# NCAR/SPERR

Measured on AMD Instinct MI355X. Metric: compress+decompress GB/s/GPU on 256^3 fp32 chunks @ BPP=2.0; bitstream-exact vs ref, higher is better.
Workload: dtype f64; 1 GPU; synthetic 1024^3 fp32 turbulence per GPU, 256^3 chunks, BPP=2.0, step = compress + decompress, volume and container resident in HBM; chunks_per_gpu=64, parallelism=chunks farmed over 1 GPU(s), no collective

## Files before the change

### sperr_amd/csrc/xform.hip

```cpp
#include <type_traits>

#include "xform.h"
#include "lift_window.h"
#include "dequant.h"

namespace sperrhip {


constexpr int kSumStrides = 64, kSumSeg = 64;


template <typename T>
__global__ void __launch_bounds__(kThreads)
k_stride_sums(const T* __restrict__ vol, VolDesc vd, const ChunkGeom* geom, uint32_t cx,
              uint32_t cy, uint32_t cz, uint32_t nstrides, uint32_t ssz, double* strideMean,
              size_t strideMeanStride, CoderState* st, int want_range)
{
  __shared__ double tile[kSumStrides][kSumSeg + 1];
  __shared__ uint32_t sh_differs;
  double vmax = -INFINITY, vnegmax = -INFINITY;
  const uint32_t c = blockIdx.y;
  const uint32_t s0 = blockIdx.x * kSumStrides;
  const ChunkGeom g = geom[c];
  const size_t vx = vd.dims[0], vy = vd.dims[1];
  const T first = vol[((size_t)g.org[2] * vy + g.org[1]) * vx + g.org[0]];
  if (threadIdx.x == 0)
    sh_differs = 0;
  double acc = 0.0;
  bool differs = false;
  (void)cz;
  for (uint32_t seg = 0; seg < ssz; seg += kSumSeg) {
    const uint32_t len = min((uint32_t)kSumSeg, ssz - seg);
    __syncthreads();
    for (uint32_t k = threadIdx.x; k < (uint32_t)(kSumStrides * kSumSeg); k += kThreads) {
      const uint32_t r = k / kSumSeg, j = k % kSumSeg;
      const uint32_t sidx = s0 + r;
      if (sidx < nstrides && j < len) {
        const uint32_t e = sidx * ssz + seg + j;
        const uint32_t x = e % cx, q = e / cx;
        const uint32_t y = q % cy, z = q / cy;
        const T v = vol[((size_t)(g.org[2] + z) * vy + (g.org[1] + y)) * vx + g.org[0] + x];
        differs |= (v != first);
        tile[r][j] = (double)v;
        vmax = fmax(vmax, (double)v);
        vnegmax = fmax(vnegmax, -(double)v);
      }
    }
    __syncthreads();
    if (threadIdx.x < (uint32_t)kSumStrides && s0 + threadIdx.x < nstrides)
      for (uint32_t j = 0; j < len; j++)
        acc += tile[threadIdx.x][j];
  }
  if (differs)
    sh_differs = 1;
  __syncthreads();
  if (threadIdx.x < (uint32_t)kSumStrides && s0 + threadIdx.x < nstrides)
    strideMean[c * strideMeanStride + s0 + threadIdx.x] = acc / (double)ssz;
  if (threadIdx.x == 0 && sh_differs)
    st[c].not_const_flag = 1;
  if (want_range) {
    for (int d = 32; d > 0; d >>= 1) {
      vmax = fmax(vmax, __shfl_xor(vmax, d, 64));
      vnegmax = fmax(vnegmax, __shfl_xor(vnegmax, d, 64));
    }
    if ((threadIdx.x & 63) == 0) {
      atomicMax(reinterpret_cast<unsigned long long*>(&st[c].vmaxKey), order_key(vmax));
      atomicMax(reinterpret_cast<unsigned long long*>(&st[c].vnegmaxKey), order_key(vnegmax));
    }
  }
}

template <typename T>
__global__ void __launch_bounds__(64)
k_stride_sums_rows(const T* __restrict__ vol, VolDesc vd, const ChunkGeom* geom, uint32_t cx,
                   uint32_t cy, uint32_t nstrides, uint32_t ssz, double* strideMean,
                   size_t strideMeanStride, CoderState* st, int want_range)
{
  constexpr int V = 16 / sizeof(T);
  struct alignas(16) Pack { T v[V]; };
  const uint32_t c = blockIdx.y;
  const uint32_t sidx = blockIdx.x * 64 + threadIdx.x;
  const ChunkGeom g = geom[c];
  const size_t vx = vd.dims[0], vy = vd.dims[1];
  const T first = vol[((size_t)g.org[2] * vy + g.org[1]) * vx + g.org[0]];
  double acc = 0.0, vmax = -INFINITY, vnegmax = -INFINITY;
  bool differs = false;
// ... 288 lines not shown
    }
    else {
      if (l < nl)
        for (uint32_t i = k0; i < odd_len; i += kg)
          OD(i) = (-K.eps) * OD(i);
      __syncthreads();
      if (l < nl)
        for (uint32_t i = k0; i < even_len; i += kg) {
          const uint32_t a = max(i, 1u) - 1, b = min(i, odd_len - 1);
          const double t = K.delta * (OD(a) + OD(b));
          EV(i) = fma(EV(i), K.inv_eps, -t);
        }
      __syncthreads();
      odd_step(-K.gamma);
      even_step(-K.beta);
      odd_step(-K.alpha);
    }
#undef EV
#undef OD
  }

  auto crop_store = [&](uint32_t l, uint32_t p, VT v) {
    uint32_t xyz[3];
    xyz[axis] = p;
    xyz[ua] = u0 + l;
    xyz[wa] = tw;
    if (crop_has(cg, xyz[0], xyz[1], xyz[2]))
      vol[crop_addr(cg, vd, xyz[0], xyz[1], xyz[2])] = v;
  };
  (void)crop_store;
  const bool wantMax = FORWARD && F.mode == 1 && !is_const;
  double vmax = 0.0;
  if (axis == 0) {
    const uint32_t nseg = (len + 63) / 64;
    for (uint32_t sg = tid / 64; sg < nl * nseg; sg += kThreads / 64) {
      const uint32_t l = sg / nseg, p = (sg % nseg) * 64 + tid % 64;
      if (p >= len)
        continue;
      const uint32_t src = FORWARD ? p : ((p & 1) ? even_len + (p >> 1) : (p >> 1));
      if constexpr (kCrop)
        crop_store(l, p, (VT)(is_const ? mean : sm[src * NLP + l] + mean));
      else if (IO != 0 && !FORWARD)
        vol[vbase + l * vsu + p * vsl] = (VT)(is_const ? mean : sm[src * NLP + l] + mean);
      else {
        const double v = sm[src * NLP + l];
        tile[l * su + p] = v;
        size_t idx;
        if (wantMax && outside_inner(l, p, idx))
          vmax = fmax(vmax, fabs(v));
      }
    }
  }
  else {
    const uint32_t l = tid % NL, k0 = tid / NL, kg = kThreads / NL;
    if (l < nl)
      for (uint32_t p = k0; p < len; p += kg) {
        const uint32_t src = FORWARD ? p : ((p & 1) ? even_len + (p >> 1) : (p >> 1));
        if constexpr (kCrop)
          crop_store(l, p, (VT)(is_const ? mean : sm[src * NLP + l] + mean));
        else if (IO != 0 && !FORWARD)
          vol[vbase + l * vsu + p * vsl] = (VT)(is_const ? mean : sm[src * NLP + l] + mean);
        else {
          const double v = sm[src * NLP + l];
          tile[l * su + p * sl] = v;
          size_t idx;
          if (wantMax && outside_inner(l, p, idx))
            vmax = fmax(vmax, fabs(v));
        }
      }
  }
  if (FORWARD && F.mode == 1) {
    for (int d = 32; d > 0; d >>= 1)
      vmax = fmax(vmax, __shfl_xor(vmax, d, 64));
    if ((tid & 63) == 0 && vmax > 0.0)
      atomicMax(reinterpret_cast<unsigned long long*>(&st[c].maxabs),
                (unsigned long long)__double_as_longlong(vmax));
  }
}

constexpr int kXYHalo = 4;
constexpr int kXYThreads = 512;
constexpr int kStage = 16;
constexpr int kSeg = 8;

__device__ __forceinline__ uint32_t reflect_index(int q, int n)
{
  const int period = 2 * (n - 1);
  q = q < 0 ? -q : q;
  if (q >= period)
    q %= period;
  return (uint32_t)(q < n ? q : period - q);
}


template <bool FORWARD, int IO, bool kCrop = false>
__global__ void __launch_bounds__(kXYThreads)
k_lift_xy(double* vals, size_t valsStride, uint32_t cx, uint32_t cy, uint32_t cz, int R,
          LiftConsts K, const CoderState* st, void* volume, VolDesc vd, const GeomOf<kCrop>* geom)
{
  static_assert(IO == 1 || IO == 2, "float or double volume");
  static_assert(!kCrop || !FORWARD, "the crop variant is a last inverse pass");
  using VT = typename std::conditional<IO == 1, float, double>::type;
  const uint32_t c = blockIdx.y;
  const bool is_const = st[c].is_const != 0;
  if (is_const && FORWARD)
    return;
  double* sm = reinterpret_cast<double*>(dyn_smem);
  const uint32_t ntile = (cy + R - 1) / R;
  const uint32_t z = blockIdx.x / ntile, y0 = (blockIdx.x % ntile) * R;
  const uint32_t ylo = y0 >= (uint32_t)kXYHalo ? y0 - kXYHalo : 0u;
  const uint32_t yhi = min(cy, y0 + R + kXYHalo);
  const uint32_t yend = min(cy, y0 + R);
  const uint32_t nrow = yhi - ylo;
  const uint32_t RS = cx + 1;
  const uint32_t xe = cx - cx / 2, ye = cy - cy / 2;
  const GeomOf<kCrop> g = geom[c];
  VT* vol = reinterpret_cast<VT*>(volume);
  const size_t vsy = vd.dims[0], vsz = (size_t)vd.dims[0] * vd.dims[1];
  size_t vbase = 0;
  uint32_t wy0 = y0, wy1 = yend, wx0 = 0, wx1 = cx;
  if constexpr (kCrop) {
    wy0 = max(y0, g.lo[1]);
    wy1 = min(yend, g.hi[1]);
    wx0 = g.lo[0];
    wx1 = g.hi[0];
    if (z - g.lo[2] >= g.hi[2] - g.lo[2] || wy0 >= wy1)
      return;
  }
  else
    vbase = (size_t)(g.org[2] + z) * vsz + (size_t)g.org[1] * vsy + g.org[0];
  auto out_at = [&](uint32_t x, uint32_t y) -> size_t {
    if constexpr (kCrop)
      return crop_addr(g, vd, x, y, z);
    else
      return vbase + (size_t)y * vsy + x;
  };
  double* buf = vals + c * valsStride + (size_t)z * cx * cy;
  const double mean = st[c].mean;
  const uint32_t tid = threadIdx.x;

  if (is_const) {
    if constexpr (kCrop) {
      const uint32_t w = wx1 - wx0;
      for (uint32_t k = tid; k < (wy1 - wy0) * w; k += kXYThreads)
        vol[out_at(wx0 + k % w, wy0 + k / w)] = (VT)mean;
    }
    else
      for (uint32_t k = tid; k < (yend - y0) * cx; k += kXYThreads)
        vol[vbase + (size_t)(y0 + k / cx) * vsy + k % cx] = (VT)mean;
    return;
  }

  const uint32_t lane = tid & 63u, wave = tid >> 6, nwaves = kXYThreads / 64;
  {
    using ST = typename std::conditional<FORWARD, VT, double>::type;
    const uint32_t nxb = (cx + 63) / 64;
    const uint32_t rowsW = nrow > wave ? (nrow - wave + nwaves - 1) / nwaves : 0;
    const uint32_t items = rowsW * nxb;
    uint32_t ri = 0, bi = 0;
    for (uint32_t m0 = 0; m0 < items; m0 += kStage) {
      ST v[kStage];
      uint32_t ri2 = ri, bi2 = bi;
#pragma unroll
      for (int u = 0; u < kStage; u++) {
        const uint32_t j = wave + nwaves * ri2, x = lane + 64 * bi2;
        v[u] = 0;
        if (m0 + u < items && x < cx) {
          const uint32_t y = ylo + j;
          if (FORWARD)
            v[u] = (ST)vol[vbase + (size_t)y * vsy + x];
          else
            v[u] = (ST)buf[(size_t)((y & 1) ? ye + (y >> 1) : (y >> 1)) * cx + ((x & 1) ? xe + (x >> 1) : (x >> 1))];
        }
        if (++bi2 == nxb) {
          bi2 = 0;
// ... 78 lines not shown
        const uint32_t dcol = (x & 1) ? xe + (x >> 1) : (x >> 1);
#pragma unroll
        for (int k = 0; k < kSeg; k++) {
          const uint32_t y = y0 + q * kSeg + k;
          if (y < yend)
            buf[(size_t)((y & 1) ? ye + (y >> 1) : (y >> 1)) * cx + dcol] = r[4 + k];
        }
      }
    }
  }
  else {
    for (uint32_t xb = 0; xb < cx; xb += cpr) {
      const uint32_t x = xb + tid % cpr, q = tid / cpr;
      const bool on = x < cx && q < nq;
      double r[16];
      if (on) {
        load_column(x, q, r);
        lift16<false>(r, K);
      }
      __syncthreads();
      if (on) {
#pragma unroll
        for (int k = 0; k < kSeg; k++) {
          const uint32_t y = y0 + q * kSeg + k;
          if (y < yend)
            sm[(size_t)(y - ylo) * RS + x] = r[4 + k];
        }
      }
    }
    __syncthreads();
    lift_x(y0 - ylo, yend - ylo);
    if constexpr (kCrop) {
      for (uint32_t y = wy0 + wave; y < wy1; y += nwaves) {
        VT* dstrow = vol + out_at(wx0, y);
        const double* srow = sm + (size_t)(y - ylo) * RS;
        for (uint32_t x = wx0 + lane; x < wx1; x += 64)
          dstrow[x - wx0] = (VT)(srow[x] + mean);
      }
    }
    else
    for (uint32_t y = y0 + wave; y < yend; y += nwaves) {
      VT* dstrow = vol + vbase + (size_t)y * vsy;
      const double* srow = sm + (size_t)(y - ylo) * RS;
      for (uint32_t x = lane; x < cx; x += 64)
        dstrow[x] = (VT)(srow[x] + mean);
    }
  }
}

#ifndef XYZ_INV_THREADS
#define XYZ_INV_THREADS 1024
#endif
#ifndef XYZ_INV_PREFETCH
#define XYZ_INV_PREFETCH 2
#endif
#ifndef XYZ_FWD_THREADS
#define XYZ_FWD_THREADS 1024
#endif
constexpr int kXYZThreadsF = XYZ_FWD_THREADS, kXYZThreadsI = XYZ_INV_THREADS;
constexpr int kXYZRows = 16;
constexpr int kXYZStaged = kXYZRows + 2 * kXYHalo;
constexpr int kXYZPosF = (4096 + kXYZThreadsF - 1) / kXYZThreadsF;
constexpr int kXYZStageF = (6144 + kXYZThreadsF - 1) / kXYZThreadsF;
constexpr int kXYZPosI = 6144 / kXYZThreadsI;
#ifndef XYZ_INV_GROUP
#define XYZ_INV_GROUP 3
#endif
constexpr int kXYZGroupI = XYZ_INV_GROUP;
#ifndef XYZ_FWD_YOUT
#define XYZ_FWD_YOUT 4
#endif
#ifndef XYZ_FWD_XOUT
#define XYZ_FWD_XOUT 8
#endif
#ifndef XYZ_INV_YOUT
#define XYZ_INV_YOUT 4
#endif
#ifndef XYZ_INV_XOUT
#define XYZ_INV_XOUT 4
#endif
#ifndef XYZ_INV_XSTORE
#define XYZ_INV_XSTORE 1
#endif
#ifndef XYZ_FWD_OFF
#define XYZ_FWD_OFF 0
#endif
#ifndef XYZ_INV_OFF
#define XYZ_INV_OFF 0
#endif
template <int MASK>
__device__ __forceinline__ bool xyz_off(int bit, uint32_t nseg)
{
  return (MASK & bit) != 0 && nseg != ~0u;
}
constexpr int kXYZOutFY = XYZ_FWD_YOUT, kXYZOutFX = XYZ_FWD_XOUT, kXYZOutIY = XYZ_INV_YOUT, kXYZOutIX = XYZ_INV_XOUT;
constexpr bool xyz_out_ok(int n) { return n == 2 || n == 4 || n == 8; }
static_assert(xyz_out_ok(kXYZOutFY) && xyz_out_ok(kXYZOutFX) && xyz_out_ok(kXYZOutIY) && xyz_out_ok(kXYZOutIX), "2, 4 or 8 outputs a task");
constexpr int kXYZBoxSlots = 48;

__host__ __device__ inline uint32_t xyz_row_stride(uint32_t cx)
{
  return ((cx + 7u) & ~7u) + 9u;
}

#define XYZ_LDS_BARRIER() asm volatile("s_waitcnt lgkmcnt(0)\n\ts_barrier" ::: "memory")

__device__ __forceinline__ void xyz_put(double* row, uint32_t x, uint32_t cx, double v)
{
  row[4 + x] = v;
  if (x - 1u < 4u)
    row[4 - x] = v;
  if (cx - 2u - x < 4u)
    row[2 * cx + 2 - x] = v;
}

template <bool FORWARD, int NT, int NOUT>
__device__ __forceinline__ void xyz_lift_x(const double* src, double* dst, uint32_t RS, uint32_t cx, uint32_t jlo,
                                           uint32_t jhi, uint32_t tid, const LiftConsts& K)
{
  const uint32_t nseg = (cx + NOUT - 1) / NOUT;
  const uint32_t ntask = (jhi - jlo) * nseg;
#pragma unroll 1
  for (uint32_t t = tid; t < ntask; t += NT) {
    const uint32_t rows = jhi - jlo, sg = t / rows, rb = jlo + (t - sg * rows);
    const double* row = src + (size_t)rb * RS + sg * NOUT;
    double r[NOUT + 8];
#pragma unroll
    for (int k = 0; k < NOUT + 8; k++)
      r[k] = row[k];
    lift_window<FORWARD, NOUT + 8>(r, K);
    double* out = dst + (size_t)rb * RS + 4 + sg * NOUT;
#pragma unroll
    for (int k = 0; k < NOUT; k++)
      if (sg * NOUT + k < cx)
        out[k] = r[4 + k];
  }
}

template <int NT, int NOUT, typename VT>
__device__ __forceinline__ void xyz_lift_x_store(const double* src, VT* vrows, size_t vsy, uint32_t RS, uint32_t cx, uint32_t jlo,
                                                 uint32_t jhi, uint32_t tid, const LiftConsts& K, double mean, bool noMean,
                                                 bool doStore)
{
  const uint32_t nseg = (cx + NOUT - 1) / NOUT;
  const uint32_t ntask = (jhi - jlo) * nseg;
#pragma unroll 1
  for (uint32_t t = tid; t < ntask; t += NT) {
    const uint32_t rows = jhi - jlo, sg = t / rows, rb = t - sg * rows;
    const double* row = src + (size_t)(jlo + rb) * RS + sg * NOUT;
    double r[NOUT + 8];
#pragma unroll
    for (int k = 0; k < NOUT + 8; k++)
      r[k] = row[k];
    lift_window<false, NOUT + 8>(r, K);
    VT* out = vrows + (size_t)rb * vsy + sg * NOUT;
    VT v[NOUT];
#pragma unroll
    for (int k = 0; k < NOUT; k++)
      v[k] = (VT)(noMean ? r[4 + k] : r[4 + k] + mean);
    if (!doStore)
      continue;
    if (sg * NOUT + NOUT <= cx) {
      typedef VT Seg __attribute__((ext_vector_type(NOUT), aligned(sizeof(VT))));
      Seg s;
#pragma unroll
      for (int k = 0; k < NOUT; k++)
        s[k] = v[k];
      *reinterpret_cast<Seg*>(out) = s;
    }
    else {
#pragma unroll
      for (int k = 0; k < NOUT; k++)
        if (sg * NOUT + k < cx)
          out[k] = v[k];
    }
  }
}

template <bool FORWARD, bool APRON, int NT, int NOUT>
__device__ __forceinline__ void xyz_lift_y(const double* src, double* dst, uint32_t RS, uint32_t cx, uint32_t nt,
                                           uint32_t tid, const LiftConsts& K)
{
  const uint32_t nq = (nt + NOUT - 1) / NOUT;
  const uint32_t ntask = nq * cx;
#pragma unroll 1
  for (uint32_t t = tid; t < ntask; t += NT) {
    const uint32_t q = t / cx, x = t - q * cx;
    const double* top = src + (size_t)(q * NOUT) * RS + 4 + x;
    double r[NOUT + 8];
#pragma unroll
    for (int k = 0; k < NOUT + 8; k++)
      r[k] = top[(size_t)k * RS];
    lift_window<FORWARD, NOUT + 8>(r, K);
#pragma unroll
    for (int k = 0; k < NOUT; k++) {
      if (q * NOUT + k < nt) {
        double* row = dst + (size_t)(4 + q * NOUT + k) * RS;
        if (APRON)
          xyz_put(row, x, cx, r[4 + k]);
        else
          row[4 + x] = r[4 + k];
      }
    }
  }
}

template <typename VT, int NPOS, int NSTG, bool L2>
__device__ __forceinline__ void xyz_fwd_body(double* buf, const uint32_t orow, const size_t sliceN, uint32_t cx, uint32_t cy,
                                             uint32_t cz, const LiftConsts& K, CoderState* stc, const VT* volc, const size_t vsy,
                                             const size_t vsz, const double mean, int wantMax, uint32_t in0, uint32_t in1,
                                             uint32_t in2, uint32_t nseg, double* box)
{
  const uint32_t tid = threadIdx.x;
  const uint32_t seg = blockIdx.x % nseg, npairsAll = (cz + 1) / 2;
  const uint32_t mA = seg == 0 ? 0u : (uint32_t)((uint64_t)npairsAll * seg / nseg);
  const uint32_t mB = seg + 1 == nseg ? npairsAll : (uint32_t)((uint64_t)npairsAll * (seg + 1) / nseg);
  const uint32_t zFirst = mA >= 6 ? 2 * (mA - 6) : 0u;
  const uint32_t zEnd = seg + 1 == nseg ? cz : 2 * mB - 1;
  const uint32_t y0 = (blockIdx.x / nseg) * kXYZRows;
  const uint32_t nt = min((uint32_t)kXYZRows, cy - y0);
  const uint32_t RS = xyz_row_stride(cx);
  double* sm = reinterpret_cast<double*>(dyn_smem);
  const uint32_t bufN = (uint32_t)kXYZStaged * RS;
  const uint32_t xe = cx - cx / 2, ye = cy - cy / 2, ze = cz - cz / 2;
  const size_t boxSlice = (size_t)in0 * in1;

  const uint32_t nstage = (uint32_t)kXYZStaged * cx;
  uint32_t pk[NSTG];
#pragma unroll
  for (int k = 0; k < NSTG; k++) {
    const uint32_t q = tid + (uint32_t)k * kXYZThreadsF;
    const uint32_t j = q / cx, x = q - j * cx;
    pk[k] = (j << 27) | (reflect_index((int)y0 - kXYHalo + (int)j, (int)cy) << 12) | x;
  }
  const uint32_t npos = nt * cx;
  uint32_t srow[NPOS], ooff[NPOS];
  uint32_t boff[L2 ? 1 : NPOS];
  uint32_t outerMask = 0;
#pragma unroll
  for (int k = 0; k < NPOS; k++) {
    const uint32_t q = tid + (uint32_t)k * kXYZThreadsF;
    const uint32_t row = q / cx, col = q - row * cx, y = y0 + row;
    srow[k] = ((row + kXYHalo) << 16) | col;
    const uint32_t drow = (y & 1) ? ye + (y >> 1) : (y >> 1), dcol = (col & 1) ? xe + (col >> 1) : (col >> 1);
    ooff[k] = drow * orow + dcol;
    if constexpr (!L2)
      boff[k] = drow * in0 + dcol;
    if (!(dcol < in0 && drow < in1))
      outerMask |= 1u << k;
  }
  double sxe[NPOS], sxo[NPOS], d1p[NPOS], e1p[NPOS], d2p[NPOS];
#pragma unroll
  for (int k = 0; k < NPOS; k++)
    sxe[k] = sxo[k] = d1p[k] = e1p[k] = d2p[k] = 0.0;
  double vmax = 0.0;
  auto emit = [&](int k, uint32_t zp, double v) {
    bool toBox = false;
    if constexpr (!L2)
      toBox = box != nullptr && zp < in2 && !((outerMask >> k) & 1u);
    if (!xyz_off<XYZ_FWD_OFF>(4, nseg))
      *(toBox ? box + ((size_t)zp * boxSlice + boff[L2 ? 0 : k]) : buf + ((size_t)zp * sliceN + ooff[k])) = v;
    if (wantMax && (((outerMask >> k) & 1u) || zp >= in2))
      vmax = fmax(vmax, fabs(v));
  };

  VT pre[NSTG];
  auto issue = [&](uint32_t z) {
    const VT* src = volc + (size_t)z * vsz;
#pragma unroll
    for (int k = 0; k < NSTG; k++) {
      if (xyz_off<XYZ_FWD_OFF>(1, nseg)) {
        pre[k] = (VT)(((pk[k] + z * 40503u) * 2654435761u) >> 20);
      }
      else {
        pre[k] = (tid + (uint32_t)k * kXYZThreadsF) < nstage
                     ? src[(size_t)((pk[k] >> 12) & 0x7fffu) * vsy + (pk[k] & 0xfffu)] : (VT)0;
      }
    }
  };
  issue(zFirst);
  for (uint32_t z = zFirst; z < zEnd; z++) {
    uint32_t RSv = RS, tidv = tid;
    asm volatile("" : "+s"(RSv), "+v"(tidv));
#pragma unroll
    for (int k = 0; k < NSTG; k++)
      asm volatile("" : "+v"(pk[k]));
#pragma unroll
    for (int k = 0; k < NPOS; k++)
      asm volatile("" : "+v"(srow[k]), "+v"(ooff[k]));
    if constexpr (!L2) {
#pragma unroll
      for (int k = 0; k < NPOS; k++)
        asm volatile("" : "+v"(boff[k]));
    }
    double* A = sm + ((z & 1) ? bufN : 0u);
    double* B = sm + ((z & 1) ? 0u : bufN);
#pragma unroll
    for (int k = 0; k < NSTG; k++)
      if ((tid + (uint32_t)k * kXYZThreadsF) < nstage)
        xyz_put(A + (pk[k] >> 27) * RSv, pk[k] & 0xfffu, cx, (double)pre[k] - mean);
    if (z + 1 < zEnd)
      issue(z + 1);
    XYZ_LDS_BARRIER();
    if (!xyz_off<XYZ_FWD_OFF>(2, nseg))
      xyz_lift_x<true, kXYZThreadsF, kXYZOutFX>(A, B, RSv, cx, 0, kXYZStaged, tidv, K);
    XYZ_LDS_BARRIER();
    if (!xyz_off<XYZ_FWD_OFF>(2, nseg))
      xyz_lift_y<true, false, kXYZThreadsF, kXYZOutFY>(B, A, RSv, cx, nt, tidv, K);
    XYZ_LDS_BARRIER();
    const uint32_t m = z >> 1;
    if (xyz_off<XYZ_FWD_OFF>(8, nseg))
      continue;
    if (z & 1) {
#pragma unroll
      for (int k = 0; k < NPOS; k++)
        if ((tid + (uint32_t)k * kXYZThreadsF) < npos)
          sxo[k] = A[(srow[k] >> 16) * RSv + 4 + (srow[k] & 0xffffu)];
    }
    else {
#pragma unroll
      for (int k = 0; k < NPOS; k++) {
        if ((tid + (uint32_t)k * kXYZThreadsF) >= npos)
          continue;
        const double v = A[(srow[k] >> 16) * RSv + 4 + (srow[k] & 0xffffu)];
        if (m >= 1) {
          const double d1n = fma(K.alpha, sxe[k] + v, sxo[k]);
          const double e1n = fma(K.beta, (m == 1 ? d1n : d1p[k]) + d1n, sxe[k]);
          if (m >= 2) {
            const double d2n = fma(K.gamma, e1p[k] + e1n, d1p[k]);
            const double e2 = K.eps * fma(K.delta, (m == 2 ? d2n : d2p[k]) + d2n, e1p[k]);
            if (m >= mA) {
              emit(k, m - 2, e2);
              emit(k, ze + m - 2, (-K.inv_eps) * d2n);
            }
            d2p[k] = d2n;
          }
          d1p[k] = d1n;
          e1p[k] = e1n;
        }
        sxe[k] = v;
      }
    }
  }
#pragma unroll
  for (int k = 0; k < NPOS; k++) {
    if ((tid + (uint32_t)k * kXYZThreadsF) >= npos || seg + 1 != nseg)
      continue;
    if ((cz & 1) == 0) {
      const uint32_t M = cz / 2 - 1;
      const double d1L = fma(K.alpha, sxe[k] + sxe[k], sxo[k]);
      const double e1M = fma(K.beta, d1p[k] + d1L, sxe[k]);
      const double d2a = fma(K.gamma, e1p[k] + e1M, d1p[k]);
      const double e2a = K.eps * fma(K.delta, d2p[k] + d2a, e1p[k]);
      const double d2L = fma(K.gamma, e1M + e1M, d1L);
      const double e2L = K.eps * fma(K.delta, d2a + d2L, e1M);
      emit(k, M - 1, e2a);
      emit(k, ze + M - 1, (-K.inv_eps) * d2a);
      emit(k, M, e2L);
      emit(k, ze + M, (-K.inv_eps) * d2L);
    }
    else {
      const uint32_t M = cz / 2;
      const double e1M = fma(K.beta, d1p[k] + d1p[k], sxe[k]);
      const double d2a = fma(K.gamma, e1p[k] + e1M, d1p[k]);
      const double e2a = K.eps * fma(K.delta, d2p[k] + d2a, e1p[k]);
      const double e2L = K.eps * fma(K.delta, d2a + d2a, e1M);
      emit(k, M - 1, e2a);
      emit(k, ze + M - 1, (-K.inv_eps) * d2a);
      emit(k, M, e2L);
    }
  }
  if (wantMax) {
    for (int d = 32; d > 0; d >>= 1)
      vmax = fmax(vmax, __shfl_xor(vmax, d, 64));
    if ((tid & 63) == 0 && vmax > 0.0)
      atomicMax(reinterpret_cast<unsigned long long*>(&stc->maxabs),
                (unsigned long long)__double_as_longlong(vmax));
  }
}

template <int IO>
__global__ void __launch_bounds__(kXYZThreadsF) __attribute__((amdgpu_waves_per_eu(kXYZThreadsF / 256, kXYZThreadsF / 256)))
k_lift_xyz_fwd(double* vals, size_t valsStride, uint32_t cx, uint32_t cy, uint32_t cz, LiftConsts K,
               CoderState* st, const void* volume, VolDesc vd, const ChunkGeom* geom, int wantMax,
               uint32_t in0, uint32_t in1, uint32_t in2, uint32_t nseg, double* box, size_t boxStride)
{
  static_assert(IO == 1 || IO == 2, "float or double volume");
  using VT = typename std::conditional<IO == 1, float, double>::type;
  const uint32_t c = blockIdx.y;
  if (st[c].is_const != 0)
    return;
  const VT* vol = reinterpret_cast<const VT*>(volume);
// ... 816 lines not shown

bool lift_xy_applicable(const uint32_t cdims[3])
{
  return xy_rows(cdims[0], cdims[1]) > 0;
}

int launch_lift_xy(hipStream_t stream, bool forward, double* vals, size_t valsStride,
                   uint32_t nchunks, const uint32_t cdims[3], const CoderState* st, int io,
                   void* volume, VolDesc vd, const ChunkGeom* geom, const CropGeom* crop)
{
  if (crop && forward)
    return -1;
  {
    const void* fns[6] = {reinterpret_cast<const void*>(&k_lift_xy<true, 1>),
                          reinterpret_cast<const void*>(&k_lift_xy<true, 2>),
                          reinterpret_cast<const void*>(&k_lift_xy<false, 1>),
                          reinterpret_cast<const void*>(&k_lift_xy<false, 2>),
                          reinterpret_cast<const void*>(&k_lift_xy<false, 1, true>),
                          reinterpret_cast<const void*>(&k_lift_xy<false, 2, true>)};
    for (const void* f : fns)
      if (set_max_dyn_lds(f, 160 * 1024))
        return -1;
  }
  const int R = xy_rows(cdims[0], cdims[1]);
  if (R <= 0 || (io != 1 && io != 2))
    return -1;
  const size_t smem = (size_t)(R + 2 * kXYHalo) * (cdims[0] + 1) * sizeof(double);
  const uint32_t ntile = (cdims[1] + R - 1) / R;
  const dim3 grid(ntile * cdims[2], nchunks);
  const LiftConsts K = lift_consts();
#define XY_ARGS vals, valsStride, cdims[0], cdims[1], cdims[2], R, K, st, volume, vd, geom
  if (forward) {
    if (io == 1)
      LAUNCH_K((k_lift_xy<true, 1>), grid, dim3(kXYThreads), smem, stream, XY_ARGS);
    else
      LAUNCH_K((k_lift_xy<true, 2>), grid, dim3(kXYThreads), smem, stream, XY_ARGS);
  }
  else if (crop) {
#define CROP_ARGS vals, valsStride, cdims[0], cdims[1], cdims[2], R, K, st, volume, vd, crop
    if (io == 1)
      LAUNCH_K((k_lift_xy<false, 1, true>), grid, dim3(kXYThreads), smem, stream, CROP_ARGS);
    else
      LAUNCH_K((k_lift_xy<false, 2, true>), grid, dim3(kXYThreads), smem, stream, CROP_ARGS);
#undef CROP_ARGS
  }
  else {
    if (io == 1)
      LAUNCH_K((k_lift_xy<false, 1>), grid, dim3(kXYThreads), smem, stream, XY_ARGS);
    else
      LAUNCH_K((k_lift_xy<false, 2>), grid, dim3(kXYThreads), smem, stream, XY_ARGS);
  }
#undef XY_ARGS
  HIP_CHECK(hipGetLastError());
  return 0;
}

bool lift_xyz_applicable(const uint32_t cdims[3])
{
  if (cdims[0] < 9 || cdims[1] < 9 || cdims[2] < 9)
    return false;
  return (size_t)kXYZStaged * cdims[0] <= (size_t)kXYZPosI * kXYZThreadsI &&
         (size_t)kXYZStaged * cdims[0] <= (size_t)kXYZStageF * kXYZThreadsF &&
         (size_t)kXYZRows * cdims[0] <= (size_t)kXYZPosF * kXYZThreadsF && cdims[0] < 4096 && cdims[1] < 32768;
}

static uint32_t xyz_segments(uint32_t ntile, uint32_t nchunks, uint32_t cz)
{
  uint32_t nseg = 1;
  while (nseg < 4 && (size_t)ntile * nchunks * nseg < 512 && cz / (2 * nseg) >= 24)
    nseg *= 2;
  return nseg;
}

int launch_lift_xyz(hipStream_t stream, bool forward, double* vals, size_t valsStride, uint32_t nchunks,
                    const uint32_t cdims[3], CoderState* st, int io, void* volume, VolDesc vd,
                    const ChunkGeom* geom, const LiftFuse* fuse, const CropGeom* crop, double* box, size_t boxStride)
{
  if (!lift_xyz_applicable(cdims) || (io != 1 && io != 2) || (crop && forward))
    return -1;
  if (box && !forward)
    return -1;
  const LiftFuse F = fuse ? *fuse : LiftFuse{};
  size_t smem = 2 * (size_t)kXYZStaged * xyz_row_stride(cdims[0]) * sizeof(double);
#if XYZ_INV_PREFETCH == 2
  if (!forward)
    smem += (size_t)kXYZThreadsI * kXYZPosI * 2 * sizeof(uint32_t) +
            (size_t)kXYZBoxSlots * 64 * sizeof(uint32_t);
#endif
  {
    const void* fns[10] = {reinterpret_cast<const void*>(&k_lift_xyz_fwd<1>), reinterpret_cast<const void*>(&k_lift_xyz_fwd<2>),
                           reinterpret_cast<const void*>(&k_lift_xyz_inv<1, false>), reinterpret_cast<const void*>(&k_lift_xyz_inv<2, false>),
                           reinterpret_cast<const void*>(&k_lift_xyz_inv<1, true>), reinterpret_cast<const void*>(&k_lift_xyz_inv<2, true>),
                           reinterpret_cast<const void*>(&k_lift_xyz_inv<1, false, true>), reinterpret_cast<const void*>(&k_lift_xyz_inv<2, false, true>),
                           reinterpret_cast<const void*>(&k_lift_xyz_inv<1, true, true>), reinterpret_cast<const void*>(&k_lift_xyz_inv<2, true, true>)};
    for (const void* f : fns)
      if (set_max_dyn_lds(f, 160 * 1024))
        return -1;
  }
  const uint32_t ntile = (cdims[1] + kXYZRows - 1) / kXYZRows;
  const uint32_t nseg = xyz_segments(ntile, nchunks, cdims[2]);
  const dim3 grid(ntile * nseg, nchunks);
  const LiftConsts K = lift_consts();
  if (forward) {
    const int wantMax = F.mode == 1 ? 1 : 0;
    if (io == 1)
      LAUNCH_K((k_lift_xyz_fwd<1>), grid, dim3(kXYZThreadsF), smem, stream, vals, valsStride, cdims[0], cdims[1],
               cdims[2], K, st, volume, vd, geom, wantMax, F.inner[0], F.inner[1], F.inner[2], nseg, box, boxStride);
    else
      LAUNCH_K((k_lift_xyz_fwd<2>), grid, dim3(kXYZThreadsF), smem, stream, vals, valsStride, cdims[0], cdims[1],
               cdims[2], K, st, volume, vd, geom, wantMax, F.inner[0], F.inner[1], F.inner[2], nseg, box, boxStride);
  }
  else {
    const bool sg = F.mode == 2 && F.src.coefSigned != 0;
#define XYZ_INV_LAUNCH(io_, sg_)                                                                                    \
  LAUNCH_K((k_lift_xyz_inv<io_, sg_>), grid, dim3(kXYZThreadsI), smem, stream, vals, valsStride, cdims[0], cdims[1], \
           cdims[2], K, st, volume, vd, geom, F, nseg)
#define XYZ_CROP_LAUNCH(io_, sg_)                                                                                   \
  LAUNCH_K((k_lift_xyz_inv<io_, sg_, true>), grid, dim3(kXYZThreadsI), smem, stream, vals, valsStride, cdims[0],      \
           cdims[1], cdims[2], K, st, volume, vd, crop, F, nseg)
    if (crop) {
      if (io == 1 && sg)
        XYZ_CROP_LAUNCH(1, true);
      else if (io == 1)
        XYZ_CROP_LAUNCH(1, false);
      else if (sg)
        XYZ_CROP_LAUNCH(2, true);
      else
        XYZ_CROP_LAUNCH(2, false);
    }
    else if (io == 1) {
      if (sg)
        XYZ_INV_LAUNCH(1, true);
      else
        XYZ_INV_LAUNCH(1, false);
    }
    else {
      if (sg)
        XYZ_INV_LAUNCH(2, true);
      else
        XYZ_INV_LAUNCH(2, false);
    }
#undef XYZ_INV_LAUNCH
#undef XYZ_CROP_LAUNCH
  }
  HIP_CHECK(hipGetLastError());
  return 0;
}

bool lift2_applicable(const uint32_t region[3])
{
  return lift_xyz_applicable(region) && region[0] <= (uint32_t)kL2MaxRow;
}

static uint32_t lift2_segments(uint32_t ntile, uint32_t nchunks, uint32_t cz)
{
  static const int forced = tune_getenv("SPERR_HIP_L2_NSEG") ? atoi(tune_getenv("SPERR_HIP_L2_NSEG")) : 0;
  if ((forced == 1 || forced == 2 || forced == 4) && cz / (2 * (uint32_t)forced) >= 8)
    return (uint32_t)forced;
  return xyz_segments(ntile, nchunks, cz);
}

int launch_lift2_fwd(hipStream_t stream, const double* box, size_t boxStride, double* vals, size_t valsStride,
                     uint32_t nchunks, const uint32_t cdims[3], const uint32_t region[3], CoderState* st,
                     const LiftFuse* fuse)
{
  if (!lift2_applicable(region) || !box || region[0] > cdims[0] || region[1] > cdims[1] || region[2] > cdims[2])
    return -1;
  const LiftFuse F = fuse ? *fuse : LiftFuse{};
  const size_t smem = 2 * (size_t)kXYZStaged * xyz_row_stride(region[0]) * sizeof(double);
  if (set_max_dyn_lds(reinterpret_cast<const void*>(&k_lift2_fwd), 160 * 1024))
    return -1;
  const uint32_t ntile = (region[1] + kXYZRows - 1) / kXYZRows;
  const uint32_t nseg = lift2_segments(ntile, nchunks, region[2]);
  LAUNCH_K(k_lift2_fwd, dim3(ntile * nseg, nchunks), dim3(kXYZThreadsF), smem, stream, box, boxStride, vals, valsStride,
           cdims[0], (size_t)cdims[0] * cdims[1], region[0], region[1], region[2], lift_consts(), st, F.mode == 1 ? 1 : 0,
           F.inner[0], F.inner[1], F.inner[2], nseg);
  HIP_CHECK(hipGetLastError());
  return 0;
}

int launch_lift2_inv(hipStream_t stream, const double* box, size_t boxStride, double* out, size_t outStride,
                     uint32_t nchunks, const uint32_t cdims[3], const uint32_t region[3], const CoderState* st,
                     const LiftFuse* fuse)
{
  if (!lift2_applicable(region) || !box || !out || !fuse || fuse->mode != 2 || region[0] > cdims[0] ||
      region[1] > cdims[1] || region[2] > cdims[2] || outStride < (size_t)region[0] * region[1] * region[2])
    return -1;
  LiftFuse F = *fuse;
  F.noMean = 1;
  size_t smem = 2 * (size_t)kXYZStaged * xyz_row_stride(region[0]) * sizeof(double);
#if XYZ_INV_PREFETCH == 2
  smem += (size_t)kXYZThreadsI * kL2PosI * 2 * sizeof(uint32_t) + (size_t)kXYZBoxSlots * 64 * sizeof(uint32_t);
#endif
  if (set_max_dyn_lds(reinterpret_cast<const void*>(&k_lift2_inv<false>), 160 * 1024) ||
      set_max_dyn_lds(reinterpret_cast<const void*>(&k_lift2_inv<true>), 160 * 1024))
    return -1;
  const uint32_t ntile = (region[1] + kXYZRows - 1) / kXYZRows;
  const uint32_t nseg = lift2_segments(ntile, nchunks, region[2]);
  const dim3 grid(ntile * nseg, nchunks);
  const LiftConsts K = lift_consts();
  if (F.src.coefSigned != 0)
    LAUNCH_K((k_lift2_inv<true>), grid, dim3(kXYZThreadsI), smem, stream, box, boxStride, region[0], region[1], region[2], K,
             st, out, outStride, F, nseg, cdims[0], (size_t)cdims[0] * cdims[1]);
  else
    LAUNCH_K((k_lift2_inv<false>), grid, dim3(kXYZThreadsI), smem, stream, box, boxStride, region[0], region[1], region[2], K,
             st, out, outStride, F, nseg, cdims[0], (size_t)cdims[0] * cdims[1]);
  HIP_CHECK(hipGetLastError());
  return 0;
}

template <typename T>
int launch_condition(hipStream_t stream, const T* vol, VolDesc vd, const ChunkGeom* geom,
                     uint32_t nchunks, const uint32_t cdims[3], uint32_t nstrides,
                     double* strideMean, size_t strideMeanStride, double* vals,
                     size_t valsStride, CoderState* st, bool gather, bool want_range,
                     bool org_x_aligned)
{
  const uint32_t n = cdims[0] * cdims[1] * cdims[2];
  const uint32_t ssz = n / nstrides;
  const uint32_t perLoad = 8 * (16 / (uint32_t)sizeof(T));
  const bool rowsPath = cdims[0] % perLoad == 0 && ssz % cdims[0] == 0 &&
                        vd.dims[0] % (16 / sizeof(T)) == 0 &&
                        reinterpret_cast<uintptr_t>(vol) % 16 == 0 && org_x_aligned;
  if (rowsPath)
    LAUNCH_K(k_stride_sums_rows<T>, dim3((nstrides + 63) / 64, nchunks), dim3(64), 0, stream, vol,
             vd, geom, cdims[0], cdims[1], nstrides, ssz, strideMean, strideMeanStride, st,
             want_range ? 1 : 0);
  else
    LAUNCH_K(k_stride_sums<T>, dim3((nstrides + kSumStrides - 1) / kSumStrides, nchunks),
             dim3(kThreads), 0, stream, vol, vd, geom, cdims[0], cdims[1], cdims[2], nstrides, ssz,
             strideMean, strideMeanStride, st, want_range ? 1 : 0);
  LAUNCH_K(k_mean_finalize<T>, dim3(nchunks), dim3(kThreads), 0, stream, vol, vd, geom,
                     nstrides, strideMean, strideMeanStride, st);
  if (gather)
    LAUNCH_K(k_gather_condition<T>, dim3((n + kThreads * 4 - 1) / (kThreads * 4), nchunks),
             dim3(kThreads), 0, stream, vol, vd, geom, cdims[0], cdims[1], n, vals, valsStride, st);
  HIP_CHECK(hipGetLastError());
  return 0;
}
template int launch_condition<float>(hipStream_t, const float*, VolDesc, const ChunkGeom*,
                                     uint32_t, const uint32_t[3], uint32_t, double*, size_t,
                                     double*, size_t, CoderState*, bool, bool, bool);
template int launch_condition<double>(hipStream_t, const double*, VolDesc, const ChunkGeom*,
                                      uint32_t, const uint32_t[3], uint32_t, double*, size_t,
                                      double*, size_t, CoderState*, bool, bool, bool);

template <typename T>
int launch_scatter(hipStream_t stream, T* vol, VolDesc vd, const ChunkGeom* geom,
                   uint32_t nchunks, const uint32_t cdims[3], const double* vals,
                   size_t valsStride, const CoderState* st, const CropGeom* crop)
{
  const uint32_t n = cdims[0] * cdims[1] * cdims[2];
// ... 96 lines not shown
```

Measured before the change: 70.68 GB/s.

## Fuse x-direction lifting into global loads in forward XYZ wavelet kernel

In the forward fused XYZ lift kernel, each thread now loads a contiguous x-window of 15 values per staged row, using vector loads where the window is interior. It runs the x lifting in registers and writes the results straight into LDS. This removes the separate LDS staging pass, one LDS barrier and the double-buffer swap for the x step, and swaps many scalar loads for wider ones. A skewed LDS row layout with extra padding is added to limit bank conflicts in the y pass. The cost is more registers per thread and a little more shared memory, which may lower occupancy; it is enabled for float input in the non-L2 path by default.

```diff
diff --git a/sperr_amd/csrc/xform.hip b/sperr_amd/csrc/xform.hip
--- a/sperr_amd/csrc/xform.hip
+++ b/sperr_amd/csrc/xform.hip
@@ -2,6 +2,7 @@
 
 #include "xform.h"
 #include "lift_window.h"
+#include "xyz_xload.h"
 #include "dequant.h"
 
 namespace sperrhip {
@@ -456,15 +457,6 @@
 constexpr int kXYThreads = 512;
 constexpr int kStage = 16;
 constexpr int kSeg = 8;
-
-__device__ __forceinline__ uint32_t reflect_index(int q, int n)
-{
-  const int period = 2 * (n - 1);
-  q = q < 0 ? -q : q;
-  if (q >= period)
-    q %= period;
-  return (uint32_t)(q < n ? q : period - q);
-}
 
 
 template <bool FORWARD, int IO, bool kCrop = false>
@@ -709,6 +701,15 @@
 #ifndef XYZ_INV_XSTORE
 #define XYZ_INV_XSTORE 1
 #endif
+#ifndef XYZ_FWD_XLOAD
+#define XYZ_FWD_XLOAD 1
+#endif
+#ifndef XYZ_FWD_XLOAD_ALONG
+#define XYZ_FWD_XLOAD_ALONG 1
+#endif
+#ifndef XYZ_FWD_XWAIT
+#define XYZ_FWD_XWAIT 1
+#endif
 #ifndef XYZ_FWD_OFF
 #define XYZ_FWD_OFF 0
 #endif
@@ -804,7 +805,7 @@
   }
 }
 
-template <bool FORWARD, bool APRON, int NT, int NOUT>
+template <bool FORWARD, bool APRON, int NT, int NOUT, bool SKEW = false>
 __device__ __forceinline__ void xyz_lift_y(const double* src, double* dst, uint32_t RS, uint32_t cx, uint32_t nt,
                                            uint32_t tid, const LiftConsts& K)
 {
@@ -813,11 +814,12 @@
 #pragma unroll 1
   for (uint32_t t = tid; t < ntask; t += NT) {
     const uint32_t q = t / cx, x = t - q * cx;
-    const double* top = src + (size_t)(q * NOUT) * RS + 4 + x;
+    const uint32_t RSs = SKEW ? RS + kXLoadPad : RS;
+    const double* top = src + (size_t)(q * NOUT) * RSs + 4 + (SKEW ? xload_skew(x) : x);
     double r[NOUT + 8];
 #pragma unroll
     for (int k = 0; k < NOUT + 8; k++)
-      r[k] = top[(size_t)k * RS];
+      r[k] = top[(size_t)k * RSs];
     lift_window<FORWARD, NOUT + 8>(r, K);
 #pragma unroll
     for (int k = 0; k < NOUT; k++) {
@@ -830,6 +832,15 @@
       }
     }
   }
+}
+
+template <typename VT, int NSTG, bool L2>
+constexpr bool xyz_fwd_xload()
+{
+  return XYZ_FWD_XLOAD != 0 && kXYZOutFX == kXLoadOut &&
+         kXYZStaged * xload_segments((uint32_t)(NSTG * kXYZThreadsF / kXYZStaged)) <= (uint32_t)kXYZThreadsF &&
+         xload_skew((uint32_t)(NSTG * kXYZThreadsF / kXYZStaged) - 1u) < (uint32_t)(NSTG * kXYZThreadsF / kXYZStaged) - 1u + kXLoadPad &&
+         (L2 ? XYZ_FWD_XLOAD >= 2 : sizeof(VT) == 4 || XYZ_FWD_XLOAD >= 3);
 }
 
 template <typename VT, int NPOS, int NSTG, bool L2>
@@ -852,13 +863,22 @@
   const uint32_t xe = cx - cx / 2, ye = cy - cy / 2, ze = cz - cz / 2;
   const size_t boxSlice = (size_t)in0 * in1;
 
-  const uint32_t nstage = (uint32_t)kXYZStaged * cx;
-  uint32_t pk[NSTG];
-#pragma unroll
-  for (int k = 0; k < NSTG; k++) {
-    const uint32_t q = tid + (uint32_t)k * kXYZThreadsF;
-    const uint32_t j = q / cx, x = q - j * cx;
-    pk[k] = (j << 27) | (reflect_index((int)y0 - kXYHalo + (int)j, (int)cy) << 12) | x;
+  constexpr bool kXL = xyz_fwd_xload<VT, NSTG, L2>();
+  constexpr int NPRE = kXL ? kXLoadFwd : NSTG;
+  const uint32_t nstage = kXL ? (uint32_t)kXYZStaged * xload_segments(cx) : (uint32_t)kXYZStaged * cx;
+  uint32_t pk[kXL ? 1 : NSTG];
+  if constexpr (kXL) {
+    uint32_t j = 0, sg = 0;
+    xload_task<XYZ_FWD_XLOAD_ALONG != 0>(tid < nstage ? tid : 0u, (uint32_t)kXYZStaged, cx, j, sg);
+    pk[0] = (j << 27) | (xload_row(y0, j, cy) << 12) | sg;
+  }
+  else {
+#pragma unroll
+    for (int k = 0; k < NSTG; k++) {
+      const uint32_t q = tid + (uint32_t)k * kXYZThreadsF;
+      const uint32_t j = q / cx, x = q - j * cx;
+      pk[k] = (j << 27) | (reflect_index((int)y0 - kXYHalo + (int)j, (int)cy) << 12) | x;
+    }
   }
   const uint32_t npos = nt * cx;
   uint32_t srow[NPOS], ooff[NPOS];
@@ -891,26 +911,73 @@
       vmax = fmax(vmax, fabs(v));
   };
 
-  VT pre[NSTG];
+  VT pre[NPRE];
   auto issue = [&](uint32_t z) {
     const VT* src = volc + (size_t)z * vsz;
-#pragma unroll
-    for (int k = 0; k < NSTG; k++) {
+    if constexpr (kXL) {
+      const uint32_t sg = pk[0] & 0xfffu;
+      const VT* row = src + (size_t)((pk[0] >> 12) & 0x7fffu) * vsy;
       if (xyz_off<XYZ_FWD_OFF>(1, nseg)) {
-        pre[k] = (VT)(((pk[k] + z * 40503u) * 2654435761u) >> 20);
-      }
-      else {
-        pre[k] = (tid + (uint32_t)k * kXYZThreadsF) < nstage
-                     ? src[(size_t)((pk[k] >> 12) & 0x7fffu) * vsy + (pk[k] & 0xfffu)] : (VT)0;
+#pragma unroll
+        for (int k = 0; k < NPRE; k++)
+          pre[k] = (VT)(((pk[0] + (uint32_t)k * 977u + z * 40503u) * 2654435761u) >> 20);
+      }
+      else if (tid < nstage) {
+        if (xload_whole(sg, cx)) {
+          constexpr int NV = 16 / (int)sizeof(VT), NFULL = NPRE / NV, NREST = NPRE - NFULL * NV;
+          typedef VT Vec __attribute__((ext_vector_type(NV), aligned(sizeof(VT))));
+          const VT* w = row + (sg * kXLoadOut - 4u);
+#pragma unroll
+          for (int g = 0; g < NFULL; g++) {
+            const Vec v = reinterpret_cast<const Vec*>(w)[g];
+#pragma unroll
+            for (int e = 0; e < NV; e++)
+              pre[g * NV + e] = v[e];
+          }
+          if constexpr (NREST == 3) {
+            typedef VT Vec3 __attribute__((ext_vector_type(3), aligned(sizeof(VT))));
+            const Vec3 v = *reinterpret_cast<const Vec3*>(w + NFULL * NV);
+            pre[NFULL * NV] = v[0], pre[NFULL * NV + 1] = v[1], pre[NFULL * NV + 2] = v[2];
+          }
+          else {
+#pragma unroll
+            for (int e = NFULL * NV; e < NPRE; e++)
+              pre[e] = w[e];
+          }
+        }
+        else {
+#pragma unroll
+          for (int k = 0; k < NPRE; k++)
+            pre[k] = row[xload_col(sg, k, cx)];
+        }
+      }
+    }
+    else {
+#pragma unroll
+      for (int k = 0; k < NSTG; k++) {
+        if (xyz_off<XYZ_FWD_OFF>(1, nseg)) {
+          pre[k] = (VT)(((pk[k] + z * 40503u) * 2654435761u) >> 20);
+        }
+        else {
+          pre[k] = (tid + (uint32_t)k * kXYZThreadsF) < nstage
+                       ? src[(size_t)((pk[k] >> 12) & 0x7fffu) * vsy + (pk[k] & 0xfffu)] : (VT)0;
+        }
       }
     }
   };
   issue(zFirst);
+#if XYZ_FWD_XWAIT
+  if constexpr (kXL) {
+#pragma unroll
+    for (int k = 0; k < NPRE; k++)
+      asm volatile("" : "+v"(pre[k]));
+  }
+#endif
   for (uint32_t z = zFirst; z < zEnd; z++) {
     uint32_t RSv = RS, tidv = tid;
     asm volatile("" : "+s"(RSv), "+v"(tidv));
 #pragma unroll
-    for (int k = 0; k < NSTG; k++)
+    for (int k = 0; k < (kXL ? 1 : NSTG); k++)
       asm volatile("" : "+v"(pk[k]));
 #pragma unroll
     for (int k = 0; k < NPOS; k++)
@@ -920,21 +987,47 @@
       for (int k = 0; k < NPOS; k++)
         asm volatile("" : "+v"(boff[k]));
     }
-    double* A = sm + ((z & 1) ? bufN : 0u);
-    double* B = sm + ((z & 1) ? 0u : bufN);
-#pragma unroll
-    for (int k = 0; k < NSTG; k++)
-      if ((tid + (uint32_t)k * kXYZThreadsF) < nstage)
-        xyz_put(A + (pk[k] >> 27) * RSv, pk[k] & 0xfffu, cx, (double)pre[k] - mean);
-    if (z + 1 < zEnd)
-      issue(z + 1);
+    double* A = sm + ((!kXL && (z & 1)) ? bufN : 0u);
+    double* B = sm + ((!kXL && (z & 1)) ? 0u : bufN);
+    if constexpr (kXL) {
+      double r[kXLoadWin];
+#pragma unroll
+      for (int k = 0; k < kXLoadWin; k++)
+        r[k] = k < NPRE ? (double)pre[k] - mean : 0.0;
+      if (z + 1 < zEnd)
+        issue(z + 1);
+      if (tid < nstage && !xyz_off<XYZ_FWD_OFF>(2, nseg)) {
+        lift_window<true, kXLoadWin>(r, K);
+        const uint32_t sg = pk[0] & 0xfffu;
+        double* out = B + (pk[0] >> 27) * (RSv + kXLoadPad) + 4 + xload_skew(sg * kXLoadOut);
+#pragma unroll
+        for (int k = 0; k < kXLoadOut; k++)
+          if (sg * kXLoadOut + k < cx)
+            out[k] = r[4 + k];
+      }
+    }
+    else {
+#pragma unroll
+      for (int k = 0; k < NSTG; k++)
+        if ((tid + (uint32_t)k * kXYZThreadsF) < nstage)
+          xyz_put(A + (pk[k] >> 27) * RSv, pk[k] & 0xfffu, cx, (double)pre[k] - mean);
+      if (z + 1 < zEnd)
+        issue(z + 1);
+      XYZ_LDS_BARRIER();
+      if (!xyz_off<XYZ_FWD_OFF>(2, nseg))
+        xyz_lift_x<true, kXYZThreadsF, kXYZOutFX>(A, B, RSv, cx, 0, kXYZStaged, tidv, K);
+    }
     XYZ_LDS_BARRIER();
     if (!xyz_off<XYZ_FWD_OFF>(2, nseg))
-      xyz_lift_x<true, kXYZThreadsF, kXYZOutFX>(A, B, RSv, cx, 0, kXYZStaged, tidv, K);
+      xyz_lift_y<true, false, kXYZThreadsF, kXYZOutFY, kXL>(B, A, RSv, cx, nt, tidv, K);
     XYZ_LDS_BARRIER();
-    if (!xyz_off<XYZ_FWD_OFF>(2, nseg))
-      xyz_lift_y<true, false, kXYZThreadsF, kXYZOutFY>(B, A, RSv, cx, nt, tidv, K);
-    XYZ_LDS_BARRIER();
+#if XYZ_FWD_XWAIT
+    if constexpr (kXL) {
+#pragma unroll
+      for (int k = 0; k < NPRE; k++)
+        asm volatile("" : "+v"(pre[k]));
+    }
+#endif
     const uint32_t m = z >> 1;
     if (xyz_off<XYZ_FWD_OFF>(8, nseg))
       continue;
@@ -1917,6 +2010,8 @@
     return -1;
   const LiftFuse F = fuse ? *fuse : LiftFuse{};
   size_t smem = 2 * (size_t)kXYZStaged * xyz_row_stride(cdims[0]) * sizeof(double);
+  if (forward)
+    smem += (size_t)kXYZStaged * kXLoadPad * sizeof(double);
 #if XYZ_INV_PREFETCH == 2
   if (!forward)
     smem += (size_t)kXYZThreadsI * kXYZPosI * 2 * sizeof(uint32_t) +
@@ -2002,7 +2097,7 @@
   if (!lift2_applicable(region) || !box || region[0] > cdims[0] || region[1] > cdims[1] || region[2] > cdims[2])
     return -1;
   const LiftFuse F = fuse ? *fuse : LiftFuse{};
-  const size_t smem = 2 * (size_t)kXYZStaged * xyz_row_stride(region[0]) * sizeof(double);
+  const size_t smem = (size_t)kXYZStaged * (2 * xyz_row_stride(region[0]) + kXLoadPad) * sizeof(double);
   if (set_max_dyn_lds(reinterpret_cast<const void*>(&k_lift2_fwd), 160 * 1024))
     return -1;
   const uint32_t ntile = (region[1] + kXYZRows - 1) / kXYZRows;
diff --git a/sperr_amd/csrc/xyz_xload.h b/sperr_amd/csrc/xyz_xload.h
--- /dev/null
+++ b/sperr_amd/csrc/xyz_xload.h
@@ -0,0 +1,69 @@
+#ifndef SPERR_AMD_XYZ_XLOAD_H
+#define SPERR_AMD_XYZ_XLOAD_H
+
+#include <cstdint>
+
+#include "xform.h"
+
+namespace sperrhip {
+
+__host__ __device__ __forceinline__ uint32_t reflect_index(int q, int n)
+{
+  const int period = 2 * (n - 1);
+  q = q < 0 ? -q : q;
+  if (q >= period)
+    q %= period;
+  return (uint32_t)(q < n ? q : period - q);
+}
+
+constexpr int kXLoadOut = 8, kXLoadWin = kXLoadOut + 8;
+constexpr int kXLoadFwd = kXLoadWin - 1;
+constexpr uint32_t kXLoadMinRow = 7;
+
+__host__ __device__ constexpr uint32_t xload_segments(uint32_t cx)
+{
+  return (cx + kXLoadOut - 1) / kXLoadOut;
+}
+
+__host__ __device__ __forceinline__ bool xload_whole(uint32_t sg, uint32_t cx)
+{
+  return sg >= 1 && kXLoadOut * sg + kXLoadOut + 4 <= cx;
+}
+
+__host__ __device__ __forceinline__ uint32_t xload_col(uint32_t sg, int k, uint32_t cx)
+{
+  int q = (int)(kXLoadOut * sg) - 4 + k;
+  q = q < 0 ? -q : q;
+  if (q >= (int)cx)
+    q = 2 * ((int)cx - 1) - q;
+  return (uint32_t)(q < 0 ? -q : q);
+}
+
+constexpr uint32_t kXLoadPad = 8;
+__host__ __device__ constexpr uint32_t xload_skew(uint32_t c)
+{
+  return c + (c >> 5);
+}
+
+__host__ __device__ __forceinline__ uint32_t xload_row(uint32_t y0, uint32_t j, uint32_t cy)
+{
+  return reflect_index((int)y0 - 4 + (int)j, (int)cy);
+}
+
+template <bool ALONG>
+__host__ __device__ __forceinline__ void xload_task(uint32_t t, uint32_t rows, uint32_t cx, uint32_t& j, uint32_t& sg)
+{
+  if (ALONG) {
+    const uint32_t ns = xload_segments(cx);
+    j = t / ns;
+    sg = t - j * ns;
+  }
+  else {
+    sg = t / rows;
+    j = t - sg * rows;
+  }
+}
+
+}
+
+#endif
```

After: 71.30 GB/s (median of 6 runs). Within noise of the previous version (+0.9%).
